# sinhvt3421/scann--material

Hardware: AMD Instinct MI355X
Metric: QM9 molecules/s forward (higher is better)
Workload: dtype f32 (projections: split-fp16 hi/lo operands, 3 v_mfma_f32_32x32x16_f16 per product, fp32 accumulate; everything else fp32)

## Files before the change

### include/scann_hip.h

```cpp
#ifndef SCANN_HIP_H
#define SCANN_HIP_H

#include <stdint.h>

#ifdef __cplusplus
extern "C" {
#endif

#define SCANN_ABI_VERSION 1

typedef enum scann_status {
  SCANN_OK = 0,
  SCANN_ERR_INVALID = -1,
  SCANN_ERR_UNSUPPORTED = -2,
  SCANN_ERR_NO_DEVICE = -3,
  SCANN_ERR_HIP = -4,
  SCANN_ERR_WEIGHTS = -5,
  SCANN_ERR_OOM = -6,
  SCANN_ERR_RANGE = -7
} scann_status;

typedef struct scann_config {
  int32_t n_atoms;
  int32_t embedding_dim;
// ... 266 lines not shown
                          int64_t* sums);

int scann_comm_unique_id(char* out128);
int scann_comm_init(scann_handle_t* h, const char* id128, int rank, int world);
int scann_comm_ranks(scann_handle_t* h);
int scann_broadcast_weights(scann_handle_t* h, int root);

int scann_models_load(scann_handle_t* h, int32_t n_models, const float* const* blobs, const scann_tensor_desc_t* const* manifests,
                      const int32_t* n_tensors, const int32_t* relu_out);
int scann_models_count(const scann_handle_t* h);
int scann_forward_models(scann_handle_t* h, scann_dbatch_t* db, int stream_slot);
int scann_models_download(scann_handle_t* h, scann_dbatch_t* db, float* y, float* ga);

const char* scann_pack_last_error(void);
int scann_pack_padded(int32_t B, int32_t M, int32_t N, const int32_t* atomic, const float* cgcnn,
                      const uint8_t* atom_mask, const int32_t* neighbors, const uint8_t* neighbor_mask,
                      const float* neighbor_weight, const float* neighbor_distance, const float* ring,
                      int32_t* out_atomic, float* out_cgcnn, float* out_ring, int32_t* out_mol_offset,
                      int32_t* out_edge_offset, int32_t* out_edge_col, float* out_edge_dist,
                      float* out_edge_weight, int32_t* out_row_of, int32_t* n_atom, int32_t* n_edge);
int scann_slice_count(const int64_t* ds_mol_offset, const int64_t* ds_edge_offset, const int64_t* sel, int32_t n_sel,
                      int64_t n_struct_total, int64_t* n_atom, int64_t* n_edge);
int scann_slice_batch(const int64_t* ds_mol_offset, const int64_t* ds_edge_offset, const int32_t* ds_atomic,
                      const float* ds_ring, const int32_t* ds_edge_local, const float* ds_edge_dist,
                      const float* ds_edge_weight, const int64_t* sel, int32_t n_sel, int64_t n_struct_total,
                      int32_t* out_atomic, float* out_ring, int32_t* out_mol_offset, int32_t* out_edge_offset,
                      int32_t* out_edge_col, float* out_edge_dist, float* out_edge_weight);
int scann_count_padded(int32_t B, int32_t M, int32_t N, const void* atom_mask, int32_t atom_mask_size, const void* neighbor_mask,
                       int32_t neighbor_mask_size, int32_t* out_mol_offset, int32_t* out_edge_offset, int32_t* out_row_of,
                       int32_t* n_atom, int32_t* n_edge);
int scann_host_copy(void* dst, const void* src, int64_t bytes);
int scann_plan_tiles(const scann_batch_t* batch, int32_t tile_rows, int32_t tile_atoms, int32_t allow_chunks, int32_t cap,
                     int32_t* tiles_out, int32_t* part_out, int32_t* n_tiles, int32_t* n_slots);

#ifdef __cplusplus
}
#endif
#endif
```

### scann--material_amd/csrc/scann_forward.cpp

```cpp
#include "scann_runtime.h"

namespace {

constexpr unsigned kTimingEventFlags = hipEventDisableSystemFence;

int ensure_debug(scann_handle* h, scann_dbatch* db) {
  const int L = h->cfg.n_attention;
  if (db->dbg_layers == L) return SCANN_OK;
  HIPCHK(h, cached_malloc((void**)&db->dbg_c, (size_t)(L + 1) * db->n_atom * D * 4));
  HIPCHK(h, cached_malloc((void**)&db->dbg_ctx, (size_t)std::max(L, 1) * db->n_atom * D * 4));
  if (h->cfg.g_update) HIPCHK(h, cached_malloc((void**)&db->dbg_g, (size_t)(L + 1) * std::max(db->n_edge, 1) * D * 4));
  db->dbg_layers = L;
  return SCANN_OK;
}

int ensure_outputs(scann_handle* h, scann_dbatch* db, const FwdOpts& o) {
  db->out_layers = o.train ? 0 : o.out_layers;
  db->out_flags = o.train ? 0 : o.out_flags;
  db->out_attn = db->out_z = db->out_bf = nullptr;
  if (!db->out_layers && !db->out_flags) return SCANN_OK;
  const scann_config_t& c = h->cfg;
  const size_t n_attn = (size_t)__builtin_popcountll(db->out_layers) * db->n_edge * c.num_head;
  const size_t n_z = db->out_flags & SCANN_OUT_AFTER_LC ? (size_t)db->n_atom * c.global_dim : 0;
  const size_t n_bf = db->out_flags & SCANN_OUT_BF_PROPERTY ? (size_t)db->n_struct * c.dense_out : 0;
// ... 383 lines not shown
    if (mc && mc->p_attn > 0.f && db->n_edge > 0) {
      ea.attn_drop_p = mc->p_attn;
      ea.attn_drop_seed = mc->seed;
      ea.attn_drop_tag = DROP_TAG_ATTN + (unsigned)l;
      ea.mc_rows = mc->rows;
      ea.mc_t = mc->t;
    }
#ifdef SCANN_STAMPS
    if (!getenv("SCANN_STAMP_ATOM") && l == (getenv("SCANN_STAMP_LAYER") ? atoi(getenv("SCANN_STAMP_LAYER")) : L - 1)) {
      if (!db->stamps) HIPCHK(h, hipMalloc((void**)&db->stamps, (size_t)db->n_tile * 16 * sizeof(unsigned long long)));
      ea.stamps = db->stamps;
      db->n_stamp = db->n_tile;
    }
#endif
    launch_edge(ea, s);
    if (nm) launch_edge_merge_set(db->big_tab, db->n_big, b.part_buf, ea.q, ea.p.ln_g, ea.p.ln_b, ea.ctx, rflag, l, nm, ast, wst, s);
    else launch_edge_merge(db->big_tab, db->n_big, b.part_buf, ea.q, ea.p.ln_g, ea.p.ln_b, ea.ctx, rflag, l, s);
    if (ea.attn_out) launch_attn_merge(db->big_tab, db->n_big, b.part_buf, db->edge_offset, db->tile_rows, ea.attn_out, s);
    if (sample) {
      (void)hipEventRecord(ev1, s);
      h->time_ev.push_back(ev0);
      h->time_ev.push_back(ev1);
      h->time_edges.push_back(db->n_edge);
    }
    if (tm) tm->mark(2);
  }
  if (!tm && !mc && !o.of_set) h->time_count++;
  ReadoutArgs r{};
  r.mol_offset = db->mol_offset; r.n_struct = db->n_struct; r.max_atoms = db->max_atoms;
  r.gq = b.gq; r.gk = b.gk; r.use_ga_norm = c.use_ga_norm; r.relu_out = W->cfg.relu_out;
  for (int m = 1; m < nm; ++m) r.relu_out |= o.members[m]->cfg.relu_out << m;
  r.p = W->head; r.ga_attn = b.ga; r.y = b.y; r.bf_out = outs ? db->out_bf : nullptr;
  r.n_member = nm; r.m_w = wst; r.m_a = ast; r.m_g = o.m_g; r.m_y = o.m_y;
  launch_readout(r, s);
  if (tm) tm->mark(3);
  HIPCHK(h, hipGetLastError());
  return SCANN_OK;
}

}

extern "C" {

int scann_forward_resident(scann_handle_t* h, scann_dbatch_t* db, int stream_slot) {
  if (!h || !db) return fail(h, SCANN_ERR_INVALID, "scann_forward_resident: null argument");
  HIPCHK(h, hipSetDevice(h->device));
  const int slot = ((stream_slot % h->nstream) + h->nstream) % h->nstream;
  db->last_slot = slot;
  return run_forward(h, db, h->streams[slot], selected_opts(h));
}

int scann_forward_profile(scann_handle_t* h, scann_dbatch_t* db, scann_profile_t* prof) {
  if (!h || !db || !prof) return fail(h, SCANN_ERR_INVALID, "scann_forward_profile: null argument");
  HIPCHK(h, hipSetDevice(h->device));
  memset(prof, 0, sizeof(*prof));
  Timer tm{h->streams[0], true, {}, {}};
  db->last_slot = 0;
  FwdOpts o = selected_opts(h);
  o.tm = &tm;
  const int r = run_forward(h, db, h->streams[0], o);
  if (r) return r;
  HIPCHK(h, hipStreamSynchronize(h->streams[0]));
  if (const int rp = check_pack_flag(h, db, "scann_forward_profile")) return rp;
  for (size_t i = 1; i < tm.ev.size(); ++i) {
    float ms = 0.f;
    (void)hipEventElapsedTime(&ms, tm.ev[i - 1], tm.ev[i]);
    switch (tm.kind[i]) {
// ... 50 lines not shown
#else
  (void)max_tiles;
  return fail(h, SCANN_ERR_UNSUPPORTED, "scann_debug_stamps: library was not built with -DSCANN_STAMPS");
#endif
}

int scann_debug_read(scann_handle_t* h, scann_dbatch_t* db, int what, int layer, float* out) {
  if (!h || !db || !out) return fail(h, SCANN_ERR_INVALID, "scann_debug_read: null argument");
  const int L = h->cfg.n_attention;
  if (db->dbg_layers != L) return fail(h, SCANN_ERR_INVALID, "scann_debug_read: forward was not run with debug on");
  HIPCHK(h, hipSetDevice(h->device));
  HIPCHK(h, hipStreamSynchronize(h->streams[db->last_slot]));
  if (const int rp = check_pack_flag(h, db, "scann_debug_read")) return rp;
  const size_t rowA = (size_t)db->n_atom * D, rowE = (size_t)db->n_edge * D;
  const float* src = nullptr;
  size_t n = 0;
  if (what == 0 && layer >= 0 && layer <= L) { src = db->dbg_c + layer * rowA; n = rowA; }
  else if (what == 1 && h->cfg.g_update && layer >= 0 && layer <= L) { src = db->dbg_g + layer * rowE; n = rowE; }
  else if (what == 2 && layer >= 1 && layer <= L) { src = db->dbg_ctx + (layer - 1) * rowA; n = rowA; }
  else if (what >= 3 && what <= 7 && db->kept && layer >= 1 && layer <= L) {
    const float* base = what == 3 ? db->keep_K : what == 4 ? db->keep_ang : what == 5 ? db->keep_V : what == 6 ? db->keep_T : db->keep_q;
    if (!base)
      return fail(h, SCANN_ERR_UNSUPPORTED, "scann_debug_read: this tensor is not kept by the training forward (selectors 4 = ang and 6 = T exist with the "
                                            "modular backward only: SCANN_TRAIN_FUSED=0; the base branch keeps no T)");
    n = what == 7 ? rowA : rowE;
    src = base + (size_t)(layer - 1) * n;
  }
  else return fail(h, SCANN_ERR_INVALID, "scann_debug_read: bad selector");
  if (n) HIPCHK(h, hipMemcpy(out, src, n * 4, hipMemcpyDeviceToHost));
  return SCANN_OK;
}

int64_t scann_exact_reruns(const scann_handle_t* h) { return h ? h->exact_reruns : -1; }

int scann_set_outputs(scann_handle_t* h, uint64_t attn_layers, int32_t flags) {
  if (!h) return SCANN_ERR_INVALID;
  const int L = h->cfg.n_attention;
  if (L < 64 && (attn_layers >> L) != 0)
    return fail(h, SCANN_ERR_INVALID, "scann_set_outputs: local_attention layer >= n_attention (" + std::to_string(L) + ")");
  if (flags & ~(SCANN_OUT_AFTER_LC | SCANN_OUT_BF_PROPERTY)) return fail(h, SCANN_ERR_INVALID, "scann_set_outputs: unknown output flag");
  h->out_layers = attn_layers;
  h->out_flags = flags;
  return SCANN_OK;
}

int64_t scann_output_read(scann_handle_t* h, scann_dbatch_t* db, int32_t what, int32_t layer, float* out, int64_t cap) {
  if (!h || !db) return fail(h, SCANN_ERR_INVALID, "scann_output_read: null argument");
  const scann_config_t& c = h->cfg;
  int64_t n = 0;
  if (what == SCANN_OUT_LOCAL_ATTENTION) {
    if (layer < 0 || layer >= c.n_attention || layer >= 64 || !((db->out_layers >> layer) & 1))
      return fail(h, SCANN_ERR_INVALID, "scann_output_read: local_attention_" + std::to_string(layer) + " was not selected for the batch's last forward");
    n = (int64_t)db->n_edge * c.num_head;
  } else if (what == SCANN_OUT_AFTER_LC || what == SCANN_OUT_BF_PROPERTY) {
    if (!(db->out_flags & what))
      return fail(h, SCANN_ERR_INVALID, std::string("scann_output_read: ") + (what == SCANN_OUT_AFTER_LC ? "after_Lc" : "bf_property") +
                                            " was not selected for the batch's last forward");
    n = what == SCANN_OUT_AFTER_LC ? (int64_t)db->n_atom * c.global_dim : (int64_t)db->n_struct * c.dense_out;
  } else {
    return fail(h, SCANN_ERR_INVALID, "scann_output_read: unknown output");
  }
  if (!out) return n;
  if (cap < n) return fail(h, SCANN_ERR_INVALID, "scann_output_read: " + std::to_string(n) + " floats do not fit a buffer of " + std::to_string(cap));
  HIPCHK(h, hipSetDevice(h->device));
  hipStream_t s = h->streams[db->last_slot];
  HIPCHK(h, hipStreamSynchronize(s));
// ... 85 lines not shown
```

### scann--material_amd/csrc/scann_internal.h

```cpp
#pragma once
#include <hip/hip_runtime.h>
#include <stdint.h>

#include <string>
#include <vector>

namespace scann {

constexpr int D = 128;
constexpr int NHEAD = 8;
constexpr int HDIM = D / NHEAD;
constexpr int NG = 20;
constexpr int LDS_STRIDE = 132;
constexpr int TE_MAX = 64;
constexpr int TA = 64;
constexpr int TQ = 24;
constexpr int WPACK = D * D;
constexpr float WSCALE = 256.f;
constexpr float WMAX = 65504.f / WSCALE;

__host__ __device__ inline float drop_scale(unsigned long long seed, unsigned tag, size_t idx, float p) {
  unsigned long long z = seed + 0x9E3779B97F4A7C15ull * (idx + 1) + ((unsigned long long)tag << 48);
  z = (z ^ (z >> 30)) * 0xBF58476D1CE4E5B9ull;
  z = (z ^ (z >> 27)) * 0x94D049BB133111EBull;
// ... 244 lines not shown
};
int gen_dw_slabs(int rows, int K, int N);
size_t gen_dw_part_floats(int rows, int K, int N);
void launch_gen_transpose(const GenTransDesc* descs, int n_desc, int max_elems, const float* W, float* WT, hipStream_t s);
void launch_gen_act_bwd(const float* dY, const float* pre, const float* row_scale, int rows, int N, float drop_p, unsigned drop_tag,
                        unsigned long long drop_seed, float* out, hipStream_t s);
void launch_gen_mul_gather(const float* a, const float* B, const int32_t* idx, const float* c, int rows, int N, float* out, hipStream_t s);
void launch_gen_relu(float* y, int n, hipStream_t s);
void launch_gen_dense_dw(const GenDwArgs& a, hipStream_t s);
int gen_ln_chunks(int rows);
void launch_gen_layernorm_bwd(const float* X, const float* res, const float* gamma, const float* dY, int rows, int N, float* dX, float* stats,
                              float* part, float* dgamma, float* dbeta, hipStream_t s);
void launch_gen_attn_bwd(const float* q, const float* K, const int32_t* edge_offset, int n_atom, int d, int H, int max_degree, const float* dctx,
                         float drop_p, unsigned drop_tag, unsigned long long drop_seed, float* dq, float* dK, hipStream_t s);
void launch_gen_pool_bwd(const int32_t* mol_offset, int n_struct, int max_atoms, const float* gq, const float* gk, int dg, int use_ga_norm,
                         const float* drep, float* dgq, float* dgk, hipStream_t s);
void launch_gen_edge_to_atom(const int32_t* edge_offset, const int32_t* in_off, const int32_t* in_edge, const float* S_out, const float* S_in,
                             const float* P_a, const float* P_b, const float* acc, int n_atom, int d, float* out, hipStream_t s);
void launch_gen_table_grad(const int32_t* atomic, int n_atom, const float* dV, int emb, int n_species, float* part, float* dTable, hipStream_t s);

struct ReadoutArgs {
  const int32_t* mol_offset;
  int32_t n_struct;
  int32_t max_atoms;
  const float *gq, *gk;
  int32_t use_ga_norm, relu_out;
  HeadParams p;
  float* ga_attn;
  float* y;
  float* bf_out;
  int32_t n_member;
  int64_t m_w, m_a, m_g, m_y;
};
void launch_readout(const ReadoutArgs& a, hipStream_t s);

struct AblateArgs {
  const int32_t* mol_offset;
  int32_t n_struct, max_atoms;
  const float *gq, *gk;
  int32_t dg, dout;
  int32_t use_ga_norm, relu_out, mode;
  const float *Wb, *bb, *wo, *bo;
  const float* ga_attn;
  float* y_abl;
  int32_t* order;
};
size_t ablate_lds_bytes(int max_atoms, int dg);
hipError_t launch_ablate(const AblateArgs& a, bool mfma, hipStream_t s);

struct ShapleyArgs {
  const int32_t* mol_offset;
  int32_t n_struct, n_atom, max_atoms, n_perm;
  const float *gq, *gk;
  int32_t dg, dout;
  int32_t use_ga_norm, relu_out;
  const float *Wb, *bb, *wo, *bo;
  unsigned long long seed;
  const unsigned long long* keys;
  const int32_t* perms_in;
  const int64_t* pair_offset;
  float* pair;
  float* values;
  int32_t* perms;
  double *shapley, *stderr_out;
  double *baseline, *full;
};
constexpr int SHAPLEY_PCHUNK = 4;
// ... 47 lines not shown
```

### scann--material_amd/csrc/scann_kernels.hip

```cpp
#include <algorithm>
#include <cstdlib>
#include <type_traits>
#include "scann_internal.h"
#include "scann_mma.h"

namespace scann {


__device__ __forceinline__ void mc_row_key(const AtomArgs& a, int atom, unsigned long long& seed, size_t& e) {
  const McRow m = a.mc_rows[atom];
  seed = mc_seed(a.drop_seed, a.mc_t, m.key);
  e = (size_t)(atom - m.a0) * D;
}
__device__ __forceinline__ float4 mc_drop4(unsigned long long seed, unsigned tag, size_t e, float p, float4 v) {
  v.x *= drop_scale(seed, tag, e, p);
  v.y *= drop_scale(seed, tag, e + 1, p);
  v.z *= drop_scale(seed, tag, e + 2, p);
  v.w *= drop_scale(seed, tag, e + 3, p);
  return v;
}
__device__ __forceinline__ float4 mc_keep4(uint32_t bits, float p, float4 v) {
  const float sc = 1.0f / (1.0f - p);
  v.x *= (bits & 1u) ? sc : 0.f;
  v.y *= (bits & 2u) ? sc : 0.f;
// ... 486 lines not shown
    const int la = i / cin, k = i % cin, at = a0 + la;
    float v;
    if (k < a.emb_dim) {
      if (a.cgcnn) {
        float acc = 0.f;
        for (int j = 0; j < 92; ++j) acc += a.cgcnn[(size_t)at * 92 + j] * a.We[j * a.emb_dim + k];
        v = acc + a.be[k];
      } else {
        v = a.emb[(size_t)a.atomic[at] * a.emb_dim + k];
      }
    } else {
      const int r = k - a.emb_dim;
      v = (a.ring[(size_t)at * 2] * a.Wr[r] + a.ring[(size_t)at * 2 + 1] * a.Wr[10 + r]) + a.br[r];
    }
    sV[la][k] = v;
  }
  __syncthreads();
  for (int la = 0; la < na; ++la) {
    float acc = 0.f;
    for (int k = 0; k < cin; ++k) acc += sV[la][k] * a.Wde[k * D + tid];
    a.c0[(size_t)(a0 + la) * D + tid] = swishf(acc + a.bde[tid]);
  }
}

void launch_embed(const EmbedArgs& a, hipStream_t s) {
  if (a.n_atom <= 0) return;
  hipLaunchKernelGGL(embed_kernel, dim3((a.n_atom + 7) / 8), dim3(128), 0, s, a);
}


__device__ __forceinline__ float wave_sum(float v) { return wave_sum64(v); }
__device__ __forceinline__ float wave_max(float v) { return wave_max64(v); }

template <bool SET = false>
__global__ __launch_bounds__(256) void readout_kernel(ReadoutArgs a) {
  extern __shared__ float sDyn[];
  __shared__ float sRep[D];
  __shared__ float sHead[D];
  __shared__ float sRed[4];
  unsigned sid = blockIdx.x;
  if constexpr (SET) {
    const unsigned m = blockIdx.x / (unsigned)a.n_struct;
    sid = blockIdx.x - m * (unsigned)a.n_struct;
    a.relu_out = (a.relu_out >> m) & 1;
    const int64_t w = (int64_t)m * a.m_w, x = (int64_t)m * a.m_a;
    a.p.Wb = set_member(a.p.Wb, w); a.p.bb = set_member(a.p.bb, w); a.p.wo = set_member(a.p.wo, w); a.p.bo = set_member(a.p.bo, w);
    a.gq = set_member(a.gq, x); a.gk = set_member(a.gk, x);
    a.ga_attn = set_member(a.ga_attn, (int64_t)m * a.m_g); a.y = set_member(a.y, (int64_t)m * a.m_y);
  }
  const int tid = threadIdx.x, lane = tid & 63, wave = tid >> 6;
  const int a0 = a.mol_offset[sid];
  const int n = a.mol_offset[sid + 1] - a0;
  const int T = (n + 31) >> 5, npad = T << 5;
  float* sPart = sDyn;
  float* sAgg = sDyn + 4 * npad;
  const float4* gq4 = reinterpret_cast<const float4*>(a.gq) + (size_t)a0 * 32;
  const float4* gk4 = reinterpret_cast<const float4*>(a.gk) + (size_t)a0 * 32;
  const int r = lane & 31, h = lane >> 5;

  for (int it = 0; it < T; ++it) {
    const int irow = it * 32 + r;
    float4 ka[4];
#pragma unroll
    for (int t = 0; t < 4; ++t)
      ka[t] = irow < n ? gk4[(size_t)irow * 32 + 8 * wave + 2 * t + h] : make_float4(0.f, 0.f, 0.f, 0.f);
    float part[16];
#pragma unroll
    for (int i = 0; i < 16; ++i) part[i] = 0.f;
    for (int jt = 0; jt < T; ++jt) {
      const int jrow = jt * 32 + r;
      f32x16 acc;
#pragma unroll
      for (int i = 0; i < 16; ++i) acc[i] = 0.f;
#pragma unroll
      for (int t = 0; t < 4; ++t) {
        const float4 qb = jrow < n ? gq4[(size_t)jrow * 32 + 8 * wave + 2 * t + h] : make_float4(0.f, 0.f, 0.f, 0.f);
        acc = __builtin_amdgcn_mfma_f32_32x32x2f32(ka[t].x, qb.x, acc, 0, 0, 0);
        acc = __builtin_amdgcn_mfma_f32_32x32x2f32(ka[t].y, qb.y, acc, 0, 0, 0);
        acc = __builtin_amdgcn_mfma_f32_32x32x2f32(ka[t].z, qb.z, acc, 0, 0, 0);
        acc = __builtin_amdgcn_mfma_f32_32x32x2f32(ka[t].w, qb.w, acc, 0, 0, 0);
      }
#pragma unroll
      for (int i = 0; i < 16; ++i) {
        const int gi = it * 32 + acc_row(i, lane);
        part[i] += (gi != jrow) ? acc[i] : 0.f;
      }
    }
#pragma unroll
    for (int i = 0; i < 16; ++i) {
      const float v = sum32(part[i]);
      if (r == 0) sPart[wave * npad + it * 32 + acc_row(i, lane)] = v;
    }
  }
  __syncthreads();
  for (int i = tid; i < n; i += 256)
    sAgg[i] = ((sPart[i] + sPart[npad + i]) + sPart[2 * npad + i]) + sPart[3 * npad + i];
  __syncthreads();
  if (wave == 0) {
    float nrm = 1.0f;
    if (a.use_ga_norm) {
      float ss = 0.f;
      for (int i = lane; i < n; i += 64) ss += sAgg[i] * sAgg[i];
      nrm = sqrtf(wave_sum(ss));
    }
    float m = -INFINITY;
    for (int i = lane; i < n; i += 64) {
      const float v = a.use_ga_norm ? sAgg[i] / nrm : sAgg[i];
      sAgg[i] = v;
      m = fmaxf(m, v);
    }
    m = wave_max(m);
    float ss = 0.f;
    for (int i = lane; i < n; i += 64) {
      const float e = expf(sAgg[i] - m);
      sAgg[i] = e;
      ss += e;
    }
    ss = wave_sum(ss);
    for (int i = lane; i < n; i += 64) {
      const float at = sAgg[i] / ss;
      sAgg[i] = at;
      a.ga_attn[a0 + i] = at;
    }
  }
  __syncthreads();
  {
    const int f = tid & (D - 1), half = tid >> 7;
    float rsum = 0.f;
    for (int i = half; i < n; i += 8) {
      float kv[4], av[4];
#pragma unroll
      for (int u = 0; u < 4; ++u) {
        const int iu = i + 2 * u;
        kv[u] = a.gk[(size_t)(a0 + min(iu, n - 1)) * D + f];
        av[u] = iu < n ? sAgg[iu] : 0.f;
      }
#pragma unroll
      for (int u = 0; u < 4; ++u) rsum += av[u] * kv[u];
    }
    if (half == 1) sRep[f] = rsum;
    __syncthreads();
    if (half == 0) sRep[f] = rsum + sRep[f];
  }
  __syncthreads();
  float part = 0.f;
  {
    const int f = tid & (D - 1), half = tid >> 7;
    float h0 = 0.f, h1 = 0.f, h2 = 0.f, h3 = 0.f;
    const float* __restrict__ wcol = a.p.Wb + (size_t)(64 * half) * D + f;
    const float* __restrict__ rp = sRep + 64 * half;
    for (int k0 = 0; k0 < 64; k0 += 16) {
      float wv[16];
#pragma unroll
      for (int u = 0; u < 16; ++u) wv[u] = wcol[(size_t)(k0 + u) * D];
#pragma unroll
      for (int u = 0; u < 16; u += 4) {
        h0 = fmaf(rp[k0 + u], wv[u], h0);
        h1 = fmaf(rp[k0 + u + 1], wv[u + 1], h1);
        h2 = fmaf(rp[k0 + u + 2], wv[u + 2], h2);
        h3 = fmaf(rp[k0 + u + 3], wv[u + 3], h3);
      }
    }
    const float hs = (h0 + h1) + (h2 + h3);
    if (half == 1) sHead[f] = hs;
    __syncthreads();
    if (half == 0) {
      const float hb = swish_exact((hs + sHead[f]) + a.p.bb[f]);
      if (a.bf_out) a.bf_out[(size_t)sid * D + f] = hb;
      part = hb * a.p.wo[f];
    }
  }
  part = wave_sum(part);
  if (lane == 0) sRed[wave] = part;
  __syncthreads();
  if (tid == 0) {
    float y = (sRed[0] + sRed[1]) + a.p.bo[0];
    if (a.relu_out) y = fmaxf(y, 0.f);
    a.y[sid] = y;
  }
}

void launch_readout(const ReadoutArgs& a, hipStream_t s) {
  if (a.n_struct <= 0) return;
  const size_t npad = (size_t)((a.max_atoms + 31) / 32) * 32;
  const size_t lds = 5 * npad * sizeof(float);
  if (a.n_member > 0) hipLaunchKernelGGL(readout_kernel<true>, dim3(a.n_struct * a.n_member), dim3(256), lds, s, a);
  else hipLaunchKernelGGL(readout_kernel<false>, dim3(a.n_struct), dim3(256), lds, s, a);
}

}
```

### scann--material_amd/csrc/scann_runtime.cpp

```cpp
#include "scann_runtime.h"

#include <mutex>

namespace {

struct BlockCache {
  std::multimap<size_t, void*> free_blocks;
  std::map<void*, size_t> size_of;
  size_t cached_bytes = 0;
};
std::map<int, BlockCache> g_block_cache;
std::mutex g_block_mu;
constexpr size_t BLOCK_CACHE_LIMIT = (size_t)16 << 30;
thread_local std::string g_create_error;

std::vector<WeightSpec> build_specs(const scann_config_t& c) {
  std::vector<WeightSpec> s;
  const int64_t d = c.local_dim, dg = c.global_dim, dout = c.dense_out, emb = c.embedding_dim;
  if (c.feature_cgcnn) {
    s.push_back({"embed_atom/kernel", 92, emb});
    s.push_back({"embed_atom/bias", emb, 0});
  } else {
    s.push_back({"embed_atom/embeddings", c.n_atoms, emb});
  }
// ... 209 lines not shown
  if (hipGetDeviceCount(&n) != hipSuccess) return 0;
  return n;
}

const char* scann_last_error(const scann_handle_t* h) { return h ? h->err.c_str() : g_create_error.c_str(); }

int scann_create(const scann_config_t* cfg, int device_id, scann_handle_t** out) {
  if (!cfg || !out) return fail(nullptr, SCANN_ERR_INVALID, "scann_create: null argument");
  *out = nullptr;
  if (cfg->n_gauss != NG) return fail(nullptr, SCANN_ERR_UNSUPPORTED, "scann_create: 20 Gaussians (custom_layers.py:39-53 as called by scann_model.py:378,384)");
  const bool generic = cfg->local_dim != D || cfg->global_dim != D || cfg->dense_out != D || cfg->num_head != NHEAD ||
                       (getenv("SCANN_GENERIC") && atoi(getenv("SCANN_GENERIC")));
  if (generic) {
    if (cfg->local_dim <= 0 || cfg->num_head <= 0 || cfg->global_dim <= 0 || cfg->dense_out <= 0 || cfg->local_dim % cfg->num_head != 0)
      return fail(nullptr, SCANN_ERR_INVALID, "scann_create: local_dim must be a positive multiple of num_head (attention.py:170-173), global_dim and dense_out positive");
    if (cfg->local_dim > 1024 || cfg->global_dim > 1024 || cfg->dense_out > 1024 || cfg->embedding_dim > 1024)
      return fail(nullptr, SCANN_ERR_UNSUPPORTED, "scann_create: widths above 1024 are not implemented");
  } else if (cfg->embedding_dim + (cfg->use_ring ? 10 : 0) > 160) {
    return fail(nullptr, SCANN_ERR_UNSUPPORTED, "scann_create: embedding_dim (+10 ring features) must be <= 160");
  }
  if (cfg->n_atoms <= 0 || cfg->embedding_dim <= 0 || cfg->n_attention < 0 || !(cfg->gaussian_d > 0))
    return fail(nullptr, SCANN_ERR_INVALID, "scann_create: bad hyper-parameter");
  int ndev = 0;
  if (hipGetDeviceCount(&ndev) != hipSuccess || ndev <= 0)
    return fail(nullptr, SCANN_ERR_NO_DEVICE, "scann_create: no HIP device visible (this library has no CPU fallback)");
  if (device_id < 0 || device_id >= ndev) return fail(nullptr, SCANN_ERR_NO_DEVICE, "scann_create: device_id out of range");
  scann_handle* h = new scann_handle();
  h->cfg = *cfg;
  h->generic = generic;
  h->device = device_id;
  h->specs = build_specs(*cfg);
  if (const char* xr = getenv("SCANN_XCD_REMAP")) h->xcd_remap = atoi(xr) != 0;
  if (const char* ar = getenv("SCANN_ATOM_ROWS")) h->atom_rows = atoi(ar);
  if (const char* fb = getenv("SCANN_FUSE_BASIS")) h->fuse_basis = atoi(fb) != 0;
  if (const char* st = getenv("SCANN_SPECIES_TABLES")) h->species_tables = atoi(st) != 0;
  if (const char* sg = getenv("SCANN_STRICT_RANGE")) h->strict_range = atoi(sg) != 0;
  if (const char* fe = getenv("SCANN_EXACT")) h->force_exact = atoi(fe) != 0;
  {
    hipDeviceProp_t prop;
    if (hipGetDeviceProperties(&prop, device_id) == hipSuccess && prop.multiProcessorCount > 0) h->n_cu = prop.multiProcessorCount;
  }
  if (const char* ns = getenv("SCANN_STREAMS")) h->nstream = std::min(MAX_STREAM, std::max(1, atoi(ns)));
  if (hipSetDevice(device_id) != hipSuccess) {
    delete h;
    return fail(nullptr, SCANN_ERR_HIP, "scann_create: hipSetDevice failed");
  }
  if (hipHostMalloc((void**)&h->range_flag, 128, hipHostMallocDefault) != hipSuccess) {
    delete h;
    return fail(nullptr, SCANN_ERR_HIP, "scann_create: hipHostMalloc failed");
  }
  for (int i = 0; i < 32; ++i) h->range_flag[i] = 0;
  for (int i = 0; i < h->nstream; ++i) {
    if (hipStreamCreateWithFlags(&h->streams[i], hipStreamNonBlocking) != hipSuccess) {
      delete h;
      return fail(nullptr, SCANN_ERR_HIP, "scann_create: hipStreamCreate failed");
    }
  }
  *out = h;
  return SCANN_OK;
}

void scann_destroy(scann_handle_t* h) {
  if (!h) return;
  (void)hipSetDevice(h->device);
  (void)hipDeviceSynchronize();
  for (int i = 0; i < MAX_STREAM; ++i)
// ... 378 lines not shown
```

### scann--material_amd/csrc/scann_runtime.h

```cpp
#pragma once
#include "../../include/scann_hip.h"
#include "scann_internal.h"
#include "scann_train.h"

#include <rccl/rccl.h>

#include <algorithm>
#include <cmath>
#include <cstdlib>
#include <cstring>
#include <map>
#include <memory>
#include <string>
#include <vector>

using namespace scann;

namespace scann {

constexpr int MAX_STREAM = 16;

hipError_t cached_malloc(void** p, size_t bytes);
void cached_free(void* p);
void cache_release(int dev);
// ... 57 lines not shown

struct Timer;
struct ModelSet;
void free_models(ModelSet* ms);

struct McState {
  const McRow* rows;
  unsigned long long seed;
  uint32_t t;
  float p_drop, p_attn;
};

}

struct scann_handle {
  scann_config_t cfg{};
  int device = 0;
  std::string err;
  hipStream_t streams[MAX_STREAM]{};
  int nstream = 2;
  std::vector<WeightSpec> specs;
  bool loaded = false;
  bool debug = false;
  uint64_t out_layers = 0;
  int32_t out_flags = 0;
  int tile_atoms = TQ;
  int n_cu = 256;
  int time_every = 0;
  int64_t time_count = 0;
  std::vector<hipEvent_t> time_ev;
  std::vector<int> time_edges;
  int xcd_remap = 1;
  int atom_rows = 0;
  int fuse_basis = 1;
  int species_tables = 1;
  bool generic = false;
  float* g_weights = nullptr;
  float* g_centres = nullptr;
  std::map<std::string, int64_t> g_off;
  std::vector<GenTransDesc> gt_descs;
  GenTransDesc* d_gt_descs = nullptr;
  std::map<std::string, int64_t> gt_off;
  float* g_WT = nullptr;
  int gt_max = 0;
  bool weights_exact = false;
  bool force_exact = false;
  bool strict_range = false;
  int64_t exact_reruns = 0;
  float* d_weights = nullptr;
  std::vector<LayerParams> layers;
  HeadParams head{};
  BasisParams basis{};
  const float* lut = nullptr;
  float *sp_c = nullptr, *sp_P1 = nullptr, *sp_P3 = nullptr, *sp_q = nullptr;
  bool sp_dirty = true;
  const float* cd = nullptr;
  EmbedArgs embed{};
  std::vector<float> host_master;
  std::vector<int64_t> spec_off;
  std::vector<RepackDesc> descs;
  size_t arena_floats = 0, o_lut = 0, o_emb = 0, o_Wde = 0, o_bde = 0;
  struct LayerT {
    const float *W1T, *W2T, *W3T, *WqT, *WkT, *Wf1T, *Wf2T;
    const _Float16 *W1Th, *W2Th, *W3Th, *WqTh, *WkTh, *Wf1Th, *Wf2Th;
  };
  std::vector<LayerT> layersT;
// ... 169 lines not shown
```

### scann--material_amd/scann/_hip.py

```python
from __future__ import annotations

import ctypes as C
import os

import numpy as np

_HERE = os.path.dirname(os.path.abspath(__file__))
LIB_PATH = os.environ.get("SCANN_HIP_LIB") or os.path.join(os.path.dirname(_HERE), "lib", "libscann_hip.so")

SCANN_OK = 0
STATUS = {0: "OK", -1: "INVALID", -2: "UNSUPPORTED", -3: "NO_DEVICE", -4: "HIP", -5: "WEIGHTS", -6: "OOM", -7: "RANGE"}


class ScannHipError(RuntimeError):
    def __init__(self, code, msg):
        super().__init__("libscann_hip: %s (%d): %s" % (STATUS.get(code, "?"), code, msg))
        self.code, self.detail = code, msg


class Config(C.Structure):
    _fields_ = [
        ("n_atoms", C.c_int32), ("embedding_dim", C.c_int32), ("local_dim", C.c_int32), ("num_head", C.c_int32),
        ("n_attention", C.c_int32), ("global_dim", C.c_int32), ("dense_out", C.c_int32), ("n_gauss", C.c_int32),
        ("gaussian_d", C.c_float), ("g_update", C.c_int32), ("use_attn_norm", C.c_int32), ("use_ga_norm", C.c_int32),
# ... 40 lines not shown
    ("scann_sync", C.c_int, [_P]),
    ("scann_num_streams", C.c_int, [_P]),
    ("scann_forward_profile", C.c_int, [_P, _P, C.POINTER(Profile)]),
    ("scann_edge_timing", C.c_int, [_P, C.c_int]),
    ("scann_edge_timing_read", C.c_int, [_P, C.POINTER(C.c_double), C.POINTER(C.c_int64), C.POINTER(C.c_double)]),
    ("scann_set_debug", C.c_int, [_P, C.c_int]),
    ("scann_debug_read", C.c_int, [_P, _P, C.c_int, C.c_int, _P]),
    ("scann_train_debug_read", C.c_int64, [_P, _P, C.c_char_p, _P, C.c_int64]),
    ("scann_debug_stamps", C.c_int, [_P, _P, _P, C.c_int]),
    ("scann_param_count", C.c_int64, [_P]),
    ("scann_train_begin", C.c_int, [_P]),
    ("scann_train_forward", C.c_int, [_P, _P, _P, C.c_float, C.c_uint64, C.POINTER(C.c_double)]),
    ("scann_train_backward", C.c_int, [_P, _P, C.c_double, C.c_int64]),
    ("scann_set_attention_dropout", C.c_int, [_P, C.c_float]),
    ("scann_set_deterministic", C.c_int, [_P, C.c_int]),
    ("scann_zero_grads", C.c_int, [_P]),
    ("scann_allreduce_grads", C.c_int, [_P]),
    ("scann_allreduce_sse", C.c_int, [_P, C.POINTER(C.c_double), C.POINTER(C.c_int64)]),
    ("scann_adam_step", C.c_int, [_P, C.c_float, C.c_float, C.c_float, C.c_float, C.c_float]),
    ("scann_train_step", C.c_int, [_P, _P, _P, C.c_float, C.c_uint64] + [C.c_float] * 5 + [C.POINTER(C.c_double), C.POINTER(C.c_int64)]),
    ("scann_train_step_begin", C.c_int, [_P, _P, _P, C.c_float, C.c_uint64] + [C.c_float] * 5),
    ("scann_train_step_end", C.c_int, [_P, C.POINTER(C.c_double), C.POINTER(C.c_int64), C.POINTER(C.c_double)]),
    ("scann_get_grads", C.c_int, [_P, _P]),
    ("scann_get_weights", C.c_int, [_P, _P]),
    ("scann_comm_unique_id", C.c_int, [C.c_char_p]),
    ("scann_comm_init", C.c_int, [_P, C.c_char_p, C.c_int, C.c_int]),
    ("scann_comm_ranks", C.c_int, [_P]),
    ("scann_broadcast_weights", C.c_int, [_P, C.c_int]),
    ("scann_pack_last_error", C.c_char_p, []),
    ("scann_pack_padded", C.c_int, [C.c_int32, C.c_int32, C.c_int32] + [_P] * 17 + [C.POINTER(C.c_int32), C.POINTER(C.c_int32)]),
    ("scann_slice_count", C.c_int, [_P, _P, _P, C.c_int32, C.c_int64, C.POINTER(C.c_int64), C.POINTER(C.c_int64)]),
    ("scann_slice_batch", C.c_int, [_P] * 8 + [C.c_int32, C.c_int64] + [_P] * 7),
    ("scann_plan_tiles", C.c_int, [C.POINTER(Batch), C.c_int32, C.c_int32, C.c_int32, C.c_int32, _P, _P, C.POINTER(C.c_int32), C.POINTER(C.c_int32)]),
    ("scann_exact_reruns", C.c_int64, [_P]),
    ("scann_device_memory", C.c_int, [_P, C.POINTER(C.c_int64), C.POINTER(C.c_int64)]),
    ("scann_batch_info", C.c_int, [_P, _P, _P]),
    ("scann_count_padded", C.c_int, [C.c_int32, C.c_int32, C.c_int32, _P, C.c_int32, _P, C.c_int32, _P, _P, _P, C.POINTER(C.c_int32), C.POINTER(C.c_int32)]),
    ("scann_upload_padded", C.c_int, [_P, C.c_int32, C.c_int32, C.c_int32, _P, _P, C.c_int32, _P, _P, C.c_int32, _P, _P, C.POINTER(_P),
                                      C.POINTER(C.c_int32), C.POINTER(C.c_int32)]),
    ("scann_batch_read_csr", C.c_int, [_P, _P, _P, _P, _P, _P, _P, _P]),
    ("scann_host_copy", C.c_int, [_P, _P, C.c_int64]),
    ("scann_set_outputs", C.c_int, [_P, C.c_uint64, C.c_int32]),
    ("scann_output_read", C.c_int64, [_P, _P, C.c_int32, C.c_int32, _P, C.c_int64]),
    ("scann_input_grads", C.c_int, [_P, _P, _P, _P, _P, _P, _P]),
    ("scann_predict_mc", C.c_int, [_P, _P, C.c_int32, C.c_uint64, _P, C.c_float, C.c_float, _P, _P, _P, _P, _P]),
    ("scann_mc_drop_scale", C.c_double, [C.c_uint64, C.c_int32, C.c_uint64, C.c_uint32, C.c_uint64, C.c_float]),
    ("scann_ablate_pooling", C.c_int, [_P, _P, C.c_int32, _P, _P, _P, _P]),
    ("scann_shapley", C.c_int, [_P, _P, C.c_int32, C.c_uint64, _P, _P, _P, _P, _P, _P, _P, _P, _P, _P]),
    ("scann_shapley_profile", C.c_int, [_P, _P, C.c_int32, C.c_uint64, _P, _P]),
    ("scann_shapley_permutation", None, [C.c_uint64, C.c_uint64, C.c_int32, C.c_int32, _P]),
    ("scann_shapley_reduce_host", C.c_int, [_P, _P, _P, C.c_int32, C.c_int32, _P, _P, _P, _P]),
    ("scann_rollout_floats", C.c_int64, [_P, _P]),
    ("scann_attention_rollout", C.c_int, [_P, _P, C.c_float, C.c_int32, C.c_int32, _P, _P, _P, _P]),
    ("scann_index_create", C.c_int, [_P, C.c_int32, C.POINTER(_P)]),
    ("scann_index_free", None, [_P, _P]),
    ("scann_index_size", C.c_int64, [_P]),
    ("scann_index_add", C.c_int, [_P, _P, _P, C.c_int64, _P, _P]),
    ("scann_index_read", C.c_int, [_P, _P, C.c_int64, C.c_int64, _P, _P, _P]),
    ("scann_index_query", C.c_int, [_P, _P, _P, C.c_int64, _P, C.c_int32, _P, _P, _P, _P]),
    ("scann_index_add_batch", C.c_int, [_P, _P, _P, C.c_int32, _P]),
    ("scann_index_query_batch", C.c_int, [_P, _P, _P, C.c_int32, _P, C.c_int32, _P, _P, _P, _P, _P, _P]),
    ("scann_knn_distsq", C.c_float, [_P, _P, C.c_int64]),
    ("scann_knn_distsq_matrix", None, [_P, C.c_int64, _P, C.c_int64, C.c_int64, _P]),
    ("scann_index_segments", C.c_int64, [_P, _P, _P, _P]),
    ("scann_index_match", C.c_int, [_P, _P, _P, _P, C.c_int64, _P, C.c_int32, C.c_int32, _P, _P, _P, _P, _P, _P, _P]),
    ("scann_index_match_batch", C.c_int, [_P, _P, _P, _P, C.c_int32, C.c_int32, _P, _P, _P, _P, _P, _P, _P, _P, _P]),
# ... 1836 lines not shown
```

Before: 2.083 million.

## Pack multiple small molecules per block in the readout kernel

```diff
diff --git a/include/scann_hip.h b/include/scann_hip.h
--- a/include/scann_hip.h
+++ b/include/scann_hip.h
@@ -322,6 +322,7 @@
 int scann_host_copy(void* dst, const void* src, int64_t bytes);
 int scann_plan_tiles(const scann_batch_t* batch, int32_t tile_rows, int32_t tile_atoms, int32_t allow_chunks, int32_t cap,
                      int32_t* tiles_out, int32_t* part_out, int32_t* n_tiles, int32_t* n_slots);
+int scann_readout_pack(int32_t n_member, int32_t max_atoms, int32_t n_struct, int32_t n_cu, int32_t force);
 
 #ifdef __cplusplus
 }
diff --git a/scann--material_amd/csrc/scann_forward.cpp b/scann--material_amd/csrc/scann_forward.cpp
--- a/scann--material_amd/csrc/scann_forward.cpp
+++ b/scann--material_amd/csrc/scann_forward.cpp
@@ -439,7 +439,7 @@
   for (int m = 1; m < nm; ++m) r.relu_out |= o.members[m]->cfg.relu_out << m;
   r.p = W->head; r.ga_attn = b.ga; r.y = b.y; r.bf_out = outs ? db->out_bf : nullptr;
   r.n_member = nm; r.m_w = wst; r.m_a = ast; r.m_g = o.m_g; r.m_y = o.m_y;
-  launch_readout(r, s);
+  launch_readout(r, s, h->n_cu, h->readout_pack);
   if (tm) tm->mark(3);
   HIPCHK(h, hipGetLastError());
   return SCANN_OK;
@@ -556,6 +556,9 @@
 }
 
 int64_t scann_exact_reruns(const scann_handle_t* h) { return h ? h->exact_reruns : -1; }
+int scann_readout_pack(int32_t n_member, int32_t max_atoms, int32_t n_struct, int32_t n_cu, int32_t force) {
+  return scann::readout_pack_width(n_member, max_atoms, n_struct, n_cu, force);
+}
 
 int scann_set_outputs(scann_handle_t* h, uint64_t attn_layers, int32_t flags) {
   if (!h) return SCANN_ERR_INVALID;
diff --git a/scann--material_amd/csrc/scann_internal.h b/scann--material_amd/csrc/scann_internal.h
--- a/scann--material_amd/csrc/scann_internal.h
+++ b/scann--material_amd/csrc/scann_internal.h
@@ -300,7 +300,16 @@
   int32_t n_member;
   int64_t m_w, m_a, m_g, m_y;
 };
-void launch_readout(const ReadoutArgs& a, hipStream_t s);
+#ifndef SCANN_READOUT_S
+#define SCANN_READOUT_S 2
+#endif
+constexpr int READOUT_PACK_S = SCANN_READOUT_S;
+constexpr int READOUT_RESIDENT = 4;
+inline int readout_pack_width(int n_member, int max_atoms, int n_struct, int n_cu, int force) {
+  if (n_member > 0 || max_atoms > 32 || force == 0) return 0;
+  return (force > 0 || n_struct > READOUT_RESIDENT * n_cu) ? READOUT_PACK_S : 0;
+}
+void launch_readout(const ReadoutArgs& a, hipStream_t s, int n_cu, int force_pack);
 
 struct AblateArgs {
   const int32_t* mol_offset;
diff --git a/scann--material_amd/csrc/scann_kernels.hip b/scann--material_amd/csrc/scann_kernels.hip
--- a/scann--material_amd/csrc/scann_kernels.hip
+++ b/scann--material_amd/csrc/scann_kernels.hip
@@ -542,6 +542,100 @@
 __device__ __forceinline__ float wave_sum(float v) { return wave_sum64(v); }
 __device__ __forceinline__ float wave_max(float v) { return wave_max64(v); }
 
+__device__ __forceinline__ void readout_rows(const float4* __restrict__ g4, int row, int n, int wave, int h, float4 (&v)[4]) {
+#pragma unroll
+  for (int t = 0; t < 4; ++t) v[t] = row < n ? g4[(size_t)row * 32 + 8 * wave + 2 * t + h] : make_float4(0.f, 0.f, 0.f, 0.f);
+}
+__device__ __forceinline__ f32x16 readout_tile(const float4 (&ka)[4], const float4 (&qb)[4]) {
+  f32x16 acc;
+#pragma unroll
+  for (int i = 0; i < 16; ++i) acc[i] = 0.f;
+#pragma unroll
+  for (int t = 0; t < 4; ++t) {
+    acc = __builtin_amdgcn_mfma_f32_32x32x2f32(ka[t].x, qb[t].x, acc, 0, 0, 0);
+    acc = __builtin_amdgcn_mfma_f32_32x32x2f32(ka[t].y, qb[t].y, acc, 0, 0, 0);
+    acc = __builtin_amdgcn_mfma_f32_32x32x2f32(ka[t].z, qb[t].z, acc, 0, 0, 0);
+    acc = __builtin_amdgcn_mfma_f32_32x32x2f32(ka[t].w, qb[t].w, acc, 0, 0, 0);
+  }
+  return acc;
+}
+__device__ __forceinline__ void readout_mask_add(float (&part)[16], const f32x16& acc, int it, int jrow, int lane) {
+#pragma clang fp contract(off)
+#pragma unroll
+  for (int i = 0; i < 16; ++i) {
+    const int gi = it * 32 + acc_row(i, lane);
+    part[i] += (gi != jrow) ? acc[i] : 0.f;
+  }
+}
+__device__ __forceinline__ void readout_row_sums(const float (&part)[16], float* sP, int lane) {
+#pragma unroll
+  for (int i = 0; i < 16; ++i) {
+    const float v = sum32(part[i]);
+    if ((lane & 31) == 0) sP[acc_row(i, lane)] = v;
+  }
+}
+__device__ __forceinline__ float readout_agg(float p0, float p1, float p2, float p3) { return ((p0 + p1) + p2) + p3; }
+__device__ __forceinline__ void readout_scores(float* sAgg, int n, int lane, int use_ga_norm, float* __restrict__ ga) {
+#pragma clang fp contract(off)
+  float nrm = 1.0f;
+  if (use_ga_norm) {
+    float ss = 0.f;
+    for (int i = lane; i < n; i += 64) ss = fmaf(sAgg[i], sAgg[i], ss);
+    nrm = sqrtf(wave_sum(ss));
+  }
+  float m = -INFINITY;
+  for (int i = lane; i < n; i += 64) {
+    const float v = use_ga_norm ? sAgg[i] / nrm : sAgg[i];
+    sAgg[i] = v;
+    m = fmaxf(m, v);
+  }
+  m = wave_max(m);
+  float ss = 0.f;
+  for (int i = lane; i < n; i += 64) {
+    const float e = expf(sAgg[i] - m);
+    sAgg[i] = e;
+    ss += e;
+  }
+  ss = wave_sum(ss);
+  for (int i = lane; i < n; i += 64) {
+    const float at = sAgg[i] / ss;
+    sAgg[i] = at;
+    ga[i] = at;
+  }
+}
+__device__ __forceinline__ void readout_rep_load(const float* __restrict__ gkf, const float* sAgg, int i, int n, float (&kv)[4], float (&av)[4]) {
+#pragma unroll
+  for (int u = 0; u < 4; ++u) {
+    const int iu = i + 2 * u;
+    kv[u] = gkf[(size_t)min(iu, n - 1) * D];
+    av[u] = iu < n ? sAgg[iu] : 0.f;
+  }
+}
+__device__ __forceinline__ float readout_rep_add(float rsum, const float (&kv)[4], const float (&av)[4]) {
+#pragma unroll
+  for (int u = 0; u < 4; ++u) rsum = fmaf(av[u], kv[u], rsum);
+  return rsum;
+}
+__device__ __forceinline__ void readout_head_step(const float (&wv)[16], const float* rp, float (&hh)[4]) {
+#pragma unroll
+  for (int u = 0; u < 16; u += 4) {
+    hh[0] = fmaf(rp[u], wv[u], hh[0]);
+    hh[1] = fmaf(rp[u + 1], wv[u + 1], hh[1]);
+    hh[2] = fmaf(rp[u + 2], wv[u + 2], hh[2]);
+    hh[3] = fmaf(rp[u + 3], wv[u + 3], hh[3]);
+  }
+}
+__device__ __forceinline__ float readout_head_sum(const float (&hh)[4]) { return (hh[0] + hh[1]) + (hh[2] + hh[3]); }
+__device__ __forceinline__ float readout_hidden(float hs0, float hs1, float bb) { return swish_exact((hs0 + hs1) + bb); }
+__device__ __forceinline__ float readout_term(float hb, float wo) {
+#pragma clang fp contract(off)
+  return hb * wo;
+}
+__device__ __forceinline__ float readout_y(float r0, float r1, float bo, int relu_out) {
+  const float y = (r0 + r1) + bo;
+  return relu_out ? fmaxf(y, 0.f) : y;
+}
+
 template <bool SET = false>
 __global__ __launch_bounds__(256) void readout_kernel(ReadoutArgs a) {
   extern __shared__ float sDyn[];
@@ -569,84 +663,32 @@
   const int r = lane & 31, h = lane >> 5;
 
   for (int it = 0; it < T; ++it) {
-    const int irow = it * 32 + r;
     float4 ka[4];
-#pragma unroll
-    for (int t = 0; t < 4; ++t)
-      ka[t] = irow < n ? gk4[(size_t)irow * 32 + 8 * wave + 2 * t + h] : make_float4(0.f, 0.f, 0.f, 0.f);
+    readout_rows(gk4, it * 32 + r, n, wave, h, ka);
     float part[16];
 #pragma unroll
     for (int i = 0; i < 16; ++i) part[i] = 0.f;
     for (int jt = 0; jt < T; ++jt) {
       const int jrow = jt * 32 + r;
-      f32x16 acc;
-#pragma unroll
-      for (int i = 0; i < 16; ++i) acc[i] = 0.f;
-#pragma unroll
-      for (int t = 0; t < 4; ++t) {
-        const float4 qb = jrow < n ? gq4[(size_t)jrow * 32 + 8 * wave + 2 * t + h] : make_float4(0.f, 0.f, 0.f, 0.f);
-        acc = __builtin_amdgcn_mfma_f32_32x32x2f32(ka[t].x, qb.x, acc, 0, 0, 0);
-        acc = __builtin_amdgcn_mfma_f32_32x32x2f32(ka[t].y, qb.y, acc, 0, 0, 0);
-        acc = __builtin_amdgcn_mfma_f32_32x32x2f32(ka[t].z, qb.z, acc, 0, 0, 0);
-        acc = __builtin_amdgcn_mfma_f32_32x32x2f32(ka[t].w, qb.w, acc, 0, 0, 0);
-      }
-#pragma unroll
-      for (int i = 0; i < 16; ++i) {
-        const int gi = it * 32 + acc_row(i, lane);
-        part[i] += (gi != jrow) ? acc[i] : 0.f;
-      }
-    }
-#pragma unroll
-    for (int i = 0; i < 16; ++i) {
-      const float v = sum32(part[i]);
-      if (r == 0) sPart[wave * npad + it * 32 + acc_row(i, lane)] = v;
-    }
-  }
-  __syncthreads();
-  for (int i = tid; i < n; i += 256)
-    sAgg[i] = ((sPart[i] + sPart[npad + i]) + sPart[2 * npad + i]) + sPart[3 * npad + i];
-  __syncthreads();
-  if (wave == 0) {
-    float nrm = 1.0f;
-    if (a.use_ga_norm) {
-      float ss = 0.f;
-      for (int i = lane; i < n; i += 64) ss += sAgg[i] * sAgg[i];
-      nrm = sqrtf(wave_sum(ss));
-    }
-    float m = -INFINITY;
-    for (int i = lane; i < n; i += 64) {
-      const float v = a.use_ga_norm ? sAgg[i] / nrm : sAgg[i];
-      sAgg[i] = v;
-      m = fmaxf(m, v);
-    }
-    m = wave_max(m);
-    float ss = 0.f;
-    for (int i = lane; i < n; i += 64) {
-      const float e = expf(sAgg[i] - m);
-      sAgg[i] = e;
-      ss += e;
-    }
-    ss = wave_sum(ss);
-    for (int i = lane; i < n; i += 64) {
-      const float at = sAgg[i] / ss;
-      sAgg[i] = at;
-      a.ga_attn[a0 + i] = at;
-    }
-  }
-  __syncthreads();
+      float4 qb[4];
+      readout_rows(gq4, jrow, n, wave, h, qb);
+      readout_mask_add(part, readout_tile(ka, qb), it, jrow, lane);
+    }
+    readout_row_sums(part, sPart + wave * npad + it * 32, lane);
+  }
+  __syncthreads();
+  for (int i = tid; i < n; i += 256) sAgg[i] = readout_agg(sPart[i], sPart[npad + i], sPart[2 * npad + i], sPart[3 * npad + i]);
+  __syncthreads();
+  if (wave == 0) readout_scores(sAgg, n, lane, a.use_ga_norm, a.ga_attn + a0);
+  __syncthreads();
+  const int f = tid & (D - 1), half = tid >> 7;
   {
-    const int f = tid & (D - 1), half = tid >> 7;
+    const float* __restrict__ gkf = a.gk + (size_t)a0 * D + f;
     float rsum = 0.f;
     for (int i = half; i < n; i += 8) {
       float kv[4], av[4];
-#pragma unroll
-      for (int u = 0; u < 4; ++u) {
-        const int iu = i + 2 * u;
-        kv[u] = a.gk[(size_t)(a0 + min(iu, n - 1)) * D + f];
-        av[u] = iu < n ? sAgg[iu] : 0.f;
-      }
-#pragma unroll
-      for (int u = 0; u < 4; ++u) rsum += av[u] * kv[u];
+      readout_rep_load(gkf, sAgg, i, n, kv, av);
+      rsum = readout_rep_add(rsum, kv, av);
     }
     if (half == 1) sRep[f] = rsum;
     __syncthreads();
@@ -655,43 +697,156 @@
   __syncthreads();
   float part = 0.f;
   {
-    const int f = tid & (D - 1), half = tid >> 7;
-    float h0 = 0.f, h1 = 0.f, h2 = 0.f, h3 = 0.f;
+    float hh[4] = {0.f, 0.f, 0.f, 0.f};
     const float* __restrict__ wcol = a.p.Wb + (size_t)(64 * half) * D + f;
     const float* __restrict__ rp = sRep + 64 * half;
     for (int k0 = 0; k0 < 64; k0 += 16) {
       float wv[16];
 #pragma unroll
       for (int u = 0; u < 16; ++u) wv[u] = wcol[(size_t)(k0 + u) * D];
-#pragma unroll
-      for (int u = 0; u < 16; u += 4) {
-        h0 = fmaf(rp[k0 + u], wv[u], h0);
-        h1 = fmaf(rp[k0 + u + 1], wv[u + 1], h1);
-        h2 = fmaf(rp[k0 + u + 2], wv[u + 2], h2);
-        h3 = fmaf(rp[k0 + u + 3], wv[u + 3], h3);
-      }
-    }
-    const float hs = (h0 + h1) + (h2 + h3);
+      readout_head_step(wv, rp + k0, hh);
+    }
+    const float hs = readout_head_sum(hh);
     if (half == 1) sHead[f] = hs;
     __syncthreads();
     if (half == 0) {
-      const float hb = swish_exact((hs + sHead[f]) + a.p.bb[f]);
+      const float hb = readout_hidden(hs, sHead[f], a.p.bb[f]);
       if (a.bf_out) a.bf_out[(size_t)sid * D + f] = hb;
-      part = hb * a.p.wo[f];
+      part = readout_term(hb, a.p.wo[f]);
     }
   }
   part = wave_sum(part);
   if (lane == 0) sRed[wave] = part;
   __syncthreads();
-  if (tid == 0) {
-    float y = (sRed[0] + sRed[1]) + a.p.bo[0];
-    if (a.relu_out) y = fmaxf(y, 0.f);
-    a.y[sid] = y;
-  }
-}
-
-void launch_readout(const ReadoutArgs& a, hipStream_t s) {
+  if (tid == 0) a.y[sid] = readout_y(sRed[0], sRed[1], a.p.bo[0], a.relu_out);
+}
+
+template <int S>
+__global__ __launch_bounds__(256) void readout_pack_kernel(ReadoutArgs a) {
+  __shared__ float sPart[S][4][32];
+  __shared__ float sAgg[S][32];
+  __shared__ float sRep[S][D];
+  __shared__ float sHead[S][D];
+  __shared__ float sRed[S][4];
+  const int tid = threadIdx.x, lane = tid & 63, r = lane & 31, h = lane >> 5;
+  const int wave = __builtin_amdgcn_readfirstlane(tid >> 6), half = wave >> 1, f = tid & (D - 1);
+  const int s0 = blockIdx.x * S;
+  const int ns = min(S, a.n_struct - s0);
+  int a0[S], n[S];
+#pragma unroll
+  for (int s = 0; s < S; ++s) {
+    a0[s] = n[s] = 0;
+    if (s < ns) {
+      a0[s] = a.mol_offset[s0 + s];
+      n[s] = a.mol_offset[s0 + s + 1] - a0[s];
+    }
+    __builtin_assume(n[s] <= 32);
+  }
+  constexpr int LB = S < 4 ? S : 4;
+#pragma unroll
+  for (int b = 0; b < S; b += LB) {
+    float4 ka[LB][4], qb[LB][4];
+#pragma unroll
+    for (int u = 0; u < LB; ++u)
+      if (b + u < ns) {
+        readout_rows(reinterpret_cast<const float4*>(a.gk) + (size_t)a0[b + u] * 32, r, n[b + u], wave, h, ka[u]);
+        readout_rows(reinterpret_cast<const float4*>(a.gq) + (size_t)a0[b + u] * 32, r, n[b + u], wave, h, qb[u]);
+      }
+#pragma unroll
+    for (int u = 0; u < LB; ++u)
+      if (b + u < ns) {
+        float part[16];
+#pragma unroll
+        for (int i = 0; i < 16; ++i) part[i] = 0.f;
+        readout_mask_add(part, readout_tile(ka[u], qb[u]), 0, r, lane);
+        readout_row_sums(part, sPart[b + u][wave], lane);
+      }
+  }
+  __syncthreads();
+#pragma unroll
+  for (int s = 0; s < S; ++s)
+    if (s < ns && (s & 3) == wave) {
+      for (int i = lane; i < n[s]; i += 64) sAgg[s][i] = readout_agg(sPart[s][0][i], sPart[s][1][i], sPart[s][2][i], sPart[s][3][i]);
+      readout_scores(sAgg[s], n[s], lane, a.use_ga_norm, a.ga_attn + a0[s]);
+    }
+  __syncthreads();
+  {
+    float rsum[S];
+    int nmax = 0;
+#pragma unroll
+    for (int s = 0; s < S; ++s) {
+      rsum[s] = 0.f;
+      nmax = max(nmax, n[s]);
+    }
+    for (int i = half; i < nmax; i += 8) {
+      float kv[S][4], av[S][4];
+#pragma unroll
+      for (int s = 0; s < S; ++s)
+        if (i < n[s]) readout_rep_load(a.gk + (size_t)a0[s] * D + f, sAgg[s], i, n[s], kv[s], av[s]);
+#pragma unroll
+      for (int s = 0; s < S; ++s)
+        if (i < n[s]) rsum[s] = readout_rep_add(rsum[s], kv[s], av[s]);
+    }
+    if (half == 1) {
+#pragma unroll
+      for (int s = 0; s < S; ++s)
+        if (s < ns) sRep[s][f] = rsum[s];
+    }
+    __syncthreads();
+    if (half == 0) {
+#pragma unroll
+      for (int s = 0; s < S; ++s)
+        if (s < ns) sRep[s][f] = rsum[s] + sRep[s][f];
+    }
+  }
+  __syncthreads();
+  float hs[S];
+  {
+    float hh[S][4];
+#pragma unroll
+    for (int s = 0; s < S; ++s) hh[s][0] = hh[s][1] = hh[s][2] = hh[s][3] = 0.f;
+    const float* __restrict__ wcol = a.p.Wb + (size_t)(64 * half) * D + f;
+    for (int k0 = 0; k0 < 64; k0 += 16) {
+      float wv[16];
+#pragma unroll
+      for (int u = 0; u < 16; ++u) wv[u] = wcol[(size_t)(k0 + u) * D];
+#pragma unroll
+      for (int s = 0; s < S; ++s)
+        if (s < ns) readout_head_step(wv, &sRep[s][64 * half + k0], hh[s]);
+    }
+#pragma unroll
+    for (int s = 0; s < S; ++s) {
+      hs[s] = readout_head_sum(hh[s]);
+      if (s < ns && half == 1) sHead[s][f] = hs[s];
+    }
+  }
+  __syncthreads();
+  {
+    const float bbf = a.p.bb[f], wof = a.p.wo[f];
+#pragma unroll
+    for (int s = 0; s < S; ++s)
+      if (s < ns) {
+        float part = 0.f;
+        if (half == 0) {
+          const float hb = readout_hidden(hs[s], sHead[s][f], bbf);
+          if (a.bf_out) a.bf_out[(size_t)(s0 + s) * D + f] = hb;
+          part = readout_term(hb, wof);
+        }
+        part = wave_sum(part);
+        if (lane == 0) sRed[s][wave] = part;
+      }
+  }
+  __syncthreads();
+  if (tid < ns) a.y[s0 + tid] = readout_y(sRed[tid][0], sRed[tid][1], a.p.bo[0], a.relu_out);
+}
+
+void launch_readout(const ReadoutArgs& a, hipStream_t s, int n_cu, int force_pack) {
   if (a.n_struct <= 0) return;
+  if (readout_pack_width(a.n_member, a.max_atoms, a.n_struct, n_cu, force_pack) > 0) {
+    constexpr int S = READOUT_PACK_S;
+    hipLaunchKernelGGL(readout_pack_kernel<S>, dim3((a.n_struct + S - 1) / S), dim3(256), 0, s, a);
+    return;
+  }
   const size_t npad = (size_t)((a.max_atoms + 31) / 32) * 32;
   const size_t lds = 5 * npad * sizeof(float);
   if (a.n_member > 0) hipLaunchKernelGGL(readout_kernel<true>, dim3(a.n_struct * a.n_member), dim3(256), lds, s, a);
diff --git a/scann--material_amd/csrc/scann_runtime.cpp b/scann--material_amd/csrc/scann_runtime.cpp
--- a/scann--material_amd/csrc/scann_runtime.cpp
+++ b/scann--material_amd/csrc/scann_runtime.cpp
@@ -265,6 +265,7 @@
   h->specs = build_specs(*cfg);
   if (const char* xr = getenv("SCANN_XCD_REMAP")) h->xcd_remap = atoi(xr) != 0;
   if (const char* ar = getenv("SCANN_ATOM_ROWS")) h->atom_rows = atoi(ar);
+  if (const char* rp = getenv("SCANN_READOUT_PACK")) h->readout_pack = atoi(rp) != 0;
   if (const char* fb = getenv("SCANN_FUSE_BASIS")) h->fuse_basis = atoi(fb) != 0;
   if (const char* st = getenv("SCANN_SPECIES_TABLES")) h->species_tables = atoi(st) != 0;
   if (const char* sg = getenv("SCANN_STRICT_RANGE")) h->strict_range = atoi(sg) != 0;
diff --git a/scann--material_amd/csrc/scann_runtime.h b/scann--material_amd/csrc/scann_runtime.h
--- a/scann--material_amd/csrc/scann_runtime.h
+++ b/scann--material_amd/csrc/scann_runtime.h
@@ -113,6 +113,7 @@
   std::vector<int> time_edges;
   int xcd_remap = 1;
   int atom_rows = 0;
+  int readout_pack = -1;
   int fuse_basis = 1;
   int species_tables = 1;
   bool generic = false;
diff --git a/scann--material_amd/scann/_hip.py b/scann--material_amd/scann/_hip.py
--- a/scann--material_amd/scann/_hip.py
+++ b/scann--material_amd/scann/_hip.py
@@ -96,6 +96,7 @@
     ("scann_slice_count", C.c_int, [_P, _P, _P, C.c_int32, C.c_int64, C.POINTER(C.c_int64), C.POINTER(C.c_int64)]),
     ("scann_slice_batch", C.c_int, [_P] * 8 + [C.c_int32, C.c_int64] + [_P] * 7),
     ("scann_plan_tiles", C.c_int, [C.POINTER(Batch), C.c_int32, C.c_int32, C.c_int32, C.c_int32, _P, _P, C.POINTER(C.c_int32), C.POINTER(C.c_int32)]),
+    ("scann_readout_pack", C.c_int, [C.c_int32, C.c_int32, C.c_int32, C.c_int32, C.c_int32]),
     ("scann_exact_reruns", C.c_int64, [_P]),
     ("scann_device_memory", C.c_int, [_P, C.POINTER(C.c_int64), C.POINTER(C.c_int64)]),
     ("scann_batch_info", C.c_int, [_P, _P, _P]),
```

Result: no change. 2.087 million, median of 2 (+0.2%).
